# mohammed-amr/detectInBlur

Measured on AMD Instinct MI355X. Metric: blurred imgs/sec @800x1333 (--gpu_blur sparse correlation, fp16, batch 8), higher is better.
Workload: dtype f16; 1 GPU; configs[1]: --gpu_blur batch=8 3x800x1333 fp16, param_index=1 (expl 0.005), low_exposure fractions {1/18,1/10,1/5}, bit-exact accumulation; batch_per_gpu=8, parallelism=image-parallel x1

## Files before the change

### detectinblur_amd/csrc/dib_blur.hip

```cpp
#include "dib_compact_dev.h"
#include <mutex>
#include <stdlib.h>
#include <string.h>

extern "C" { __device__ __attribute__((used)) unsigned *dib_status_word = nullptr; }
#define DIB_STATUS_HANDOFF 1u
#define DIB_STATUS_GEOMETRY 2u
#define DIB_STATUS_WORDS 16
#ifdef DIB_STEP_POLLSTATS
extern "C" { __device__ __attribute__((used)) unsigned dib_poll_stats[4] = {0, 0, 0, 0}; }
#endif

namespace dib {

__device__ __forceinline__ void report_and_exit(unsigned code, unsigned detail) {
  typedef __attribute__((address_space(1))) unsigned gu32;
  gu32 *st = (gu32 *)(size_t)*(unsigned *volatile *)&dib_status_word;
  __hip_atomic_store(st + 1, detail, __ATOMIC_RELAXED, __HIP_MEMORY_SCOPE_SYSTEM);
  __hip_atomic_store(st, code, __ATOMIC_RELAXED, __HIP_MEMORY_SCOPE_SYSTEM);
  __builtin_amdgcn_endpgm();
}

typedef _Float16 h2 __attribute__((ext_vector_type(2)));
typedef unsigned uvec2 __attribute__((ext_vector_type(2)));
// ... 330 lines not shown

__device__ __forceinline__ bool band_entry(int T, int x, int t, int &local) {
  const int lo = (x * T) >> 3, hi = ((x + 1) * T) >> 3;
  local = lo + t;
  return t < hi - lo;
}
__device__ __forceinline__ void tile_of_local(const ImageDesc &d, int local, int &ch, int &tx, int &ty) {
  const int per_ch = d.tiles_x * d.tiles_y;
  ch = magic_div(local, d.inv_per_ch);
  local -= ch * per_ch;
  ty = magic_div(local, d.inv_tiles_x);
  tx = local - ty * d.tiles_x;
}
__device__ __forceinline__ bool tile_of_entry(const ImageDesc &d, int list, int entry, int &ch, int &tx, int &ty) {
  int local;
  if (!band_entry(d.C * d.tiles_x * d.tiles_y, list, entry, local)) return false;
  tile_of_local(d, local, ch, tx, ty);
  return true;
}
__device__ __forceinline__ void pin_desc(const ImageDesc &d) {
  asm volatile("" ::"s"(d.in), "s"(d.out), "s"(d.C), "s"(d.H), "s"(d.W), "s"(d.table), "s"(d.tiles_x), "s"(d.tiles_y),
               "s"(d.inv_per_ch), "s"(d.inv_tiles_x), "s"(d.tab));
}

constexpr int QTILE_W = 128;
constexpr int QPITCH = QUAD_PITCH * 8;
constexpr int QLDS_BYTES = LROWS * QPITCH;
static_assert(QPITCH == 448, "the asm below hard-codes the LDS row pitch");
static_assert(LROWS % NW == 0, "every wave fills the same number of window rows");
template <bool L> struct QGeom {
  static constexpr int PITCH_EL = L ? QUAD_PITCH_L : QUAD_PITCH;
  static constexpr int PITCH = PITCH_EL * 8;
  static constexpr int ROWS = TH + (L ? SEG_ROWS_L : SEG_ROWS);
  static constexpr int GQ = ROWS / NW;
  static constexpr int BYTES = ROWS * PITCH;
};
static_assert(QGeom<false>::PITCH == QPITCH && QGeom<false>::ROWS == LROWS && QGeom<false>::BYTES == QLDS_BYTES, "standard geometry");
static_assert(QGeom<true>::PITCH == 768 && QGeom<true>::ROWS % NW == 0 && QGeom<true>::BYTES == 39936, "the asm below hard-codes the large window's row pitch");

#define DIBQ_ADD(B, k) "v_pk_add_f16 %" #k ", %" #k ", v[" #B "+" #k "]\n\t"
#define DIBQ_MUL(B, k, W) "v_pk_mul_f16 v[" #B "+" #k "], " W ", v[" #B "+" #k "] op_sel:[1,0] op_sel_hi:[1,1]\n\t"
#define DIBQ_FMA(B, k, W) "v_pk_fma_f16 %" #k ", " W ", v[" #B "+" #k "], %" #k " op_sel:[1,0,0] op_sel_hi:[1,1,1]\n\t"
#define DIBQ_MADD(B, W) DIBQ_MUL(B, 0, W) DIBQ_MUL(B, 1, W) DIBQ_MUL(B, 2, W) DIBQ_MUL(B, 3, W) DIBQ_MUL(B, 4, W) DIBQ_MUL(B, 5, W) DIBQ_MUL(B, 6, W) DIBQ_MUL(B, 7, W) \
  DIBQ_ADD(B, 0) DIBQ_ADD(B, 1) DIBQ_ADD(B, 2) DIBQ_ADD(B, 3) DIBQ_ADD(B, 4) DIBQ_ADD(B, 5) DIBQ_ADD(B, 6) DIBQ_ADD(B, 7)
#define DIBQ_FMADD(B, W) DIBQ_FMA(B, 0, W) DIBQ_FMA(B, 1, W) DIBQ_FMA(B, 2, W) DIBQ_FMA(B, 3, W) DIBQ_FMA(B, 4, W) DIBQ_FMA(B, 5, W) DIBQ_FMA(B, 6, W) DIBQ_FMA(B, 7, W)
#define DIBQ_MADDH(B, W) DIBQ_MUL(B, 0, W) DIBQ_MUL(B, 2, W) DIBQ_MUL(B, 4, W) DIBQ_MUL(B, 6, W) DIBQ_ADD(B, 0) DIBQ_ADD(B, 2) DIBQ_ADD(B, 4) DIBQ_ADD(B, 6)
#define DIBQ_FMADDH(B, W) DIBQ_FMA(B, 0, W) DIBQ_FMA(B, 2, W) DIBQ_FMA(B, 4, W) DIBQ_FMA(B, 6, W)
#define DIBQ_READ(base, OFF, ADDR, P1, P2, P3)                                                                \
  "v_mad_u32_u16 v48, " OFF ", 1, " ADDR "\n\t"                                                               \
  "ds_read_b64 v[" #base ":" #base "+1], v48\n\tds_read_b64 v[" #base "+2:" #base "+3], v48 offset:" P1 "\n\t"  \
  "ds_read_b64 v[" #base "+4:" #base "+5], v48 offset:" P2 "\n\tds_read_b64 v[" #base "+6:" #base "+7], v48 offset:" P3 "\n\t"
#define DIBQ_READH(base, OFF, ADDR, P1, P2, P3)                                                               \
  "v_mad_u32_u16 v48, " OFF ", 1, " ADDR "\n\t"                                                               \
  "ds_read_b32 v[" #base "], v48\n\tds_read_b32 v[" #base "+2], v48 offset:" P1 "\n\t"                         \
  "ds_read_b32 v[" #base "+4], v48 offset:" P2 "\n\tds_read_b32 v[" #base "+6], v48 offset:" P3 "\n\t"
#define DIBQ_PITCH "448", "896", "1344"
#define DIBQ_PITCH_L "768", "1536", "2304"
#define DIBQ_LOAD(PAIR, LT, TOFF) "s_load_dwordx2 " PAIR ", " LT ", " TOFF "\n\ts_add_u32 " TOFF ", " TOFF ", 8\n\t"
#define DIBQ_NEXT(CNT, LABEL) "s_sub_u32 " CNT ", " CNT ", 1\n\ts_cbranch_scc1 " LABEL "\n\t"
#define DIBQ_LOOP6(PFX, TOFF, CNT, LT, ARITH, RD, ...) \
  DIBQ_LOAD("s[36:37]", LT, TOFF) DIBQ_LOAD("s[38:39]", LT, TOFF) "s_waitcnt vmcnt(0) lgkmcnt(0)\n\t" RD(32, "s36", __VA_ARGS__) \
  "L" PFX "_loop%=:\n\t" \
  "s_waitcnt lgkmcnt(0)\n\t" DIBQ_LOAD("s[40:41]", LT, TOFF) RD(40, "s37", __VA_ARGS__) ARITH(32, "s36") DIBQ_NEXT(CNT, "L" PFX "_done%=") \
  "s_waitcnt lgkmcnt(0)\n\t" RD(32, "s38", __VA_ARGS__) ARITH(40, "s37") DIBQ_NEXT(CNT, "L" PFX "_done%=") \
  "s_waitcnt lgkmcnt(0)\n\t" DIBQ_LOAD("s[36:37]", LT, TOFF) RD(40, "s39", __VA_ARGS__) ARITH(32, "s38") DIBQ_NEXT(CNT, "L" PFX "_done%=") \
  "s_waitcnt lgkmcnt(0)\n\t" RD(32, "s40", __VA_ARGS__) ARITH(40, "s39") DIBQ_NEXT(CNT, "L" PFX "_done%=") \
  "s_waitcnt lgkmcnt(0)\n\t" DIBQ_LOAD("s[38:39]", LT, TOFF) RD(40, "s41", __VA_ARGS__) ARITH(32, "s40") DIBQ_NEXT(CNT, "L" PFX "_done%=") \
  "s_waitcnt lgkmcnt(0)\n\t" RD(32, "s36", __VA_ARGS__) ARITH(40, "s41") \
  "s_sub_u32 " CNT ", " CNT ", 1\n\ts_cbranch_scc0 L" PFX "_loop%=\n\t" \
  "L" PFX "_done%=:\n\t" \
  "s_waitcnt lgkmcnt(0)"
#define DIBQ_CLOBBERS \
  "v32", "v33", "v34", "v35", "v36", "v37", "v38", "v39", "v40", "v41", "v42", "v43", "v44", "v45", "v46", "v47", "v48", \
  "s36", "s37", "s38", "s39", "s40", "s41", "scc", "memory"
template <bool FUSED, bool HALF, bool L = false>
__device__ __forceinline__ void tap_loop_quad(h2 (&acc)[8], unsigned long long ltaps, int t0, int n, unsigned lane_addr) {
#ifdef DIB_PORTABLE_TAPS
  return portable_taps<FUSED, HALF, 4, L ? 768u : 448u>(acc, ltaps, t0, n, lane_addr);
#endif
  unsigned toff = (unsigned)__builtin_amdgcn_readfirstlane(t0 * 4), cnt = (unsigned)__builtin_amdgcn_readfirstlane(n - 1);
  unsigned a[8];
#pragma unroll
  for (int i = 0; i < 8; ++i) a[i] = __builtin_bit_cast(unsigned, acc[i]);
#define DIB_RQ_ASM(ARITH, RD, ...) \
  asm volatile(DIBQ_LOOP6("dibq", "%8", "%9", "%10", ARITH, RD, "%11", __VA_ARGS__) \
      : "+v"(a[0]), "+v"(a[1]), "+v"(a[2]), "+v"(a[3]), "+v"(a[4]), "+v"(a[5]), "+v"(a[6]), "+v"(a[7]), "+s"(toff), "+s"(cnt) \
      : "s"(ltaps), "v"(lane_addr) \
      : DIBQ_CLOBBERS)
#define DIB_RQ_PICK(...) \
  if constexpr (FUSED && HALF) { DIB_RQ_ASM(DIBQ_FMADDH, DIBQ_READH, __VA_ARGS__); } \
  else if constexpr (FUSED) { DIB_RQ_ASM(DIBQ_FMADD, DIBQ_READ, __VA_ARGS__); } \
  else if constexpr (HALF) { DIB_RQ_ASM(DIBQ_MADDH, DIBQ_READH, __VA_ARGS__); } \
  else { DIB_RQ_ASM(DIBQ_MADD, DIBQ_READ, __VA_ARGS__); }
  if constexpr (L) { DIB_RQ_PICK(DIBQ_PITCH_L) } else { DIB_RQ_PICK(DIBQ_PITCH) }
#undef DIB_RQ_PICK
#undef DIB_RQ_ASM
#pragma unroll
  for (int i = 0; i < 8; ++i) acc[i] = __builtin_bit_cast(h2, a[i]);
}

#define DIBF_MIX(B, k, i, hs, W) "v_fma_mix_f32 %" #i ", " W ", v[" #B "+" #k "], %" #i " op_sel:[1," #hs ",0] op_sel_hi:[1,1,0]\n\t"
#define DIBF_ROWS(B, W) DIBF_MIX(B, 0, 0, 0, W) DIBF_MIX(B, 0, 1, 1, W) DIBF_MIX(B, 1, 2, 0, W) DIBF_MIX(B, 1, 3, 1, W) DIBF_MIX(B, 2, 4, 0, W) DIBF_MIX(B, 2, 5, 1, W) DIBF_MIX(B, 3, 6, 0, W) DIBF_MIX(B, 3, 7, 1, W) \
  DIBF_MIX(B, 4, 8, 0, W) DIBF_MIX(B, 4, 9, 1, W) DIBF_MIX(B, 5, 10, 0, W) DIBF_MIX(B, 5, 11, 1, W) DIBF_MIX(B, 6, 12, 0, W) DIBF_MIX(B, 6, 13, 1, W) DIBF_MIX(B, 7, 14, 0, W) DIBF_MIX(B, 7, 15, 1, W)
#define DIBF_ROWSH(B, W) DIBF_MIX(B, 0, 0, 0, W) DIBF_MIX(B, 0, 1, 1, W) DIBF_MIX(B, 2, 4, 0, W) DIBF_MIX(B, 2, 5, 1, W) DIBF_MIX(B, 4, 8, 0, W) DIBF_MIX(B, 4, 9, 1, W) DIBF_MIX(B, 6, 12, 0, W) DIBF_MIX(B, 6, 13, 1, W)
template <bool HALF, bool L>
__device__ __forceinline__ void tap_loop_quad_fp32(float (&acc)[16], unsigned long long ltaps, int t0, int n, unsigned lane_addr) {
#ifdef DIB_PORTABLE_TAPS
  {
    constexpr unsigned PITCH_B = L ? 768u : 448u;
    const unsigned *lt = reinterpret_cast<const unsigned *>(ltaps);
    for (int t = t0; t < t0 + n; ++t) {
      const unsigned word = lt[t];
      const float w = (float)half_of(word >> 16);
      const unsigned at = lane_addr + (word & 0xffffu);
#pragma unroll
      for (int i = 0; i < 4; ++i) {
        uvec2 e;
        if constexpr (HALF) { e.x = lds_b32(at + PITCH_B * i); e.y = 0; } else e = lds_b64(at + PITCH_B * i);
        acc[4 * i] = __builtin_fmaf(w, (float)half_of(e.x), acc[4 * i]);
        acc[4 * i + 1] = __builtin_fmaf(w, (float)half_of(e.x >> 16), acc[4 * i + 1]);
        if constexpr (!HALF) {
          acc[4 * i + 2] = __builtin_fmaf(w, (float)half_of(e.y), acc[4 * i + 2]);
          acc[4 * i + 3] = __builtin_fmaf(w, (float)half_of(e.y >> 16), acc[4 * i + 3]);
        }
      }
    }
    return;
  }
#endif
  unsigned toff = (unsigned)__builtin_amdgcn_readfirstlane(t0 * 4), cnt = (unsigned)__builtin_amdgcn_readfirstlane(n - 1);
#define DIB_RF_ASM(ARITH, RD, ...) \
  asm volatile(DIBQ_LOOP6("dibf", "%16", "%17", "%18", ARITH, RD, "%19", __VA_ARGS__) \
      : "+v"(acc[0]), "+v"(acc[1]), "+v"(acc[2]), "+v"(acc[3]), "+v"(acc[4]), "+v"(acc[5]), "+v"(acc[6]), "+v"(acc[7]), "+v"(acc[8]), \
        "+v"(acc[9]), "+v"(acc[10]), "+v"(acc[11]), "+v"(acc[12]), "+v"(acc[13]), "+v"(acc[14]), "+v"(acc[15]), "+s"(toff), "+s"(cnt) \
      : "s"(ltaps), "v"(lane_addr) \
      : DIBQ_CLOBBERS)
  if constexpr (L && HALF) { DIB_RF_ASM(DIBF_ROWSH, DIBQ_READH, DIBQ_PITCH_L); }
  else if constexpr (L) { DIB_RF_ASM(DIBF_ROWS, DIBQ_READ, DIBQ_PITCH_L); }
  else if constexpr (HALF) { DIB_RF_ASM(DIBF_ROWSH, DIBQ_READH, DIBQ_PITCH); }
  else { DIB_RF_ASM(DIBF_ROWS, DIBQ_READ, DIBQ_PITCH); }
#undef DIB_RF_ASM
}

#define VR_LO "op_sel:[0,0,0] op_sel_hi:[0,1,1]"
#define VR_HI "op_sel:[1,0,0] op_sel_hi:[1,1,1]"
#define VR_FMA(i, W, SEL, B, k) "v_pk_fma_f16 %" #i ", " W ", v[" #B "+" #k "], %" #i " " SEL "\n\t"
#define VR_TAP(B, j, W, SEL) VR_FMA(0, W, SEL, B, 2*j) VR_FMA(1, W, SEL, B, 2*j+1) VR_FMA(2, W, SEL, B, 2*j+2) VR_FMA(3, W, SEL, B, 2*j+3) \
  VR_FMA(4, W, SEL, B, 2*j+4) VR_FMA(5, W, SEL, B, 2*j+5) VR_FMA(6, W, SEL, B, 2*j+6) VR_FMA(7, W, SEL, B, 2*j+7)
#define VR_TAPH(B, j, W, SEL) VR_FMA(0, W, SEL, B, 2*j) VR_FMA(2, W, SEL, B, 2*j+2) VR_FMA(4, W, SEL, B, 2*j+4) VR_FMA(6, W, SEL, B, 2*j+6)
#define VR_RD(B, k, off) "ds_read_b64 v[" #B "+2*" #k ":" #B "+2*" #k "+1], v60 offset:" #off "\n\t"
#define VR_RDH(B, k, off) "ds_read_b32 v[" #B "+2*" #k "], v60 offset:" #off "\n\t"
#define VR_READS4(RD, B, OFF) "v_mad_u32_u16 v60, " OFF ", 1, %10\n\t" RD(B, 0, 0) RD(B, 1, 448) RD(B, 2, 896) RD(B, 3, 1344) RD(B, 4, 1792) RD(B, 5, 2240) RD(B, 6, 2688)
#define VR_READS3(RD, B, OFF) "v_mad_u32_u16 v60, " OFF ", 1, %10\n\t" RD(B, 0, 0) RD(B, 1, 448) RD(B, 2, 896) RD(B, 3, 1344) RD(B, 4, 1792) RD(B, 5, 2240)
#define VR_READS2(RD, B, OFF) "v_mad_u32_u16 v60, " OFF ", 1, %10\n\t" RD(B, 0, 0) RD(B, 1, 448) RD(B, 2, 896) RD(B, 3, 1344) RD(B, 4, 1792)
#define VR_READS1(RD, B, OFF) "v_mad_u32_u16 v60, " OFF ", 1, %10\n\t" RD(B, 0, 0) RD(B, 1, 448) RD(B, 2, 896) RD(B, 3, 1344)
#define VR_ARITH4(TAP, B, W01, W23) TAP(B, 3, W23, VR_HI) TAP(B, 2, W23, VR_LO) TAP(B, 1, W01, VR_HI) TAP(B, 0, W01, VR_LO)
#define VR_ARITH3(TAP, B, W01, W23) TAP(B, 2, W23, VR_LO) TAP(B, 1, W01, VR_HI) TAP(B, 0, W01, VR_LO)
#define VR_ARITH2(TAP, B, W01, W23) TAP(B, 1, W01, VR_HI) TAP(B, 0, W01, VR_LO)
#define VR_ARITH1(TAP, B, W01, W23) TAP(B, 0, W01, VR_LO)
#define VR_STEP(N, NM1, RD, TAP, BC, BN, C0, C1, C2, OTHER, P, Q)                                            \
  "Lvr_c" #N P "%=:\n\t"                                                                                    \
  "s_waitcnt lgkmcnt(0)\n\t"                                                                                \
  "s_load_dwordx4 " OTHER ", %9, %8\n\ts_add_u32 %8, %8, 16\n\t"                                            \
  VR_READS##N(RD, BN, C0)                                                                                   \
  "s_bfe_u32 s46, " C0 ", 0x30010\n\t"                                                                      \
  VR_ARITH##N(TAP, BC, C1, C2)                                                                              \
  "s_cmp_eq_u32 s46, " NM1 "\n\ts_cbranch_scc1 Lvr_c" #N Q "%=\n\t"                                         \
  "s_branch Lvr_d" Q "%=\n\t"
#define VR_BODY(N, NM1, RD, TAP)                                                                             \
  VR_STEP(N, NM1, RD, TAP, 32, 46, "s36", "s37", "s38", "s[40:43]", "x", "y")                               \
  VR_STEP(N, NM1, RD, TAP, 46, 32, "s40", "s41", "s42", "s[36:39]", "y", "x")
#define VR_DISPATCH(P)                                                                                       \
  "Lvr_d" P "%=:\n\t"                                                                                       \
  "s_cmp_eq_u32 s46, 4\n\ts_cbranch_scc1 Lvr_done%=\n\t"                                                    \
  "s_cmp_eq_u32 s46, 3\n\ts_cbranch_scc1 Lvr_c4" P "%=\n\t"                                                 \
  "s_cmp_eq_u32 s46, 2\n\ts_cbranch_scc1 Lvr_c3" P "%=\n\t"                                                 \
  "s_cmp_eq_u32 s46, 1\n\ts_cbranch_scc1 Lvr_c2" P "%=\n\t"                                                 \
  "s_branch Lvr_c1" P "%=\n\t"
template <bool HALF>
__device__ __forceinline__ void tap_loop_quad_vrun(h2 (&acc)[8], unsigned long long vgroups, int g0, unsigned lane_addr) {
#ifdef DIB_PORTABLE_TAPS
  {
    const uint4 *rec = reinterpret_cast<const uint4 *>(vgroups) + g0;
    uint4 r = rec[0];
    unsigned off = r.w & 0xffffu, code = (r.w >> 16) & 7u;
    for (int g = 0;; ++g) {
      const int n = (int)code + 1;
      uvec2 row[7];
#pragma unroll
      for (int k = 0; k < 7; ++k) {
        row[k] = uvec2{0u, 0u};
        if (k < n + 3) { if constexpr (HALF) row[k].x = lds_b32(lane_addr + off + 448u * k); else row[k] = lds_b64(lane_addr + off + 448u * k); }
      }
#pragma unroll
      for (int j = 3; j >= 0; --j) {
        if (j >= n) continue;
        const _Float16 w = half_of((j < 2 ? r.y : r.z) >> (16 * (j & 1)));
#pragma unroll
        for (int i = 0; i < 4; ++i) {
          acc[2 * i] = tap_pk<true>(acc[2 * i], row[j + i].x, w);
          if constexpr (!HALF) acc[2 * i + 1] = tap_pk<true>(acc[2 * i + 1], row[j + i].y, w);
        }
      }
      off = r.x & 0xffffu; code = (r.x >> 16) & 7u;
      if (code == 4u) break;
      r = rec[g + 1];
    }
    return;
  }
#endif
  unsigned toff = (unsigned)__builtin_amdgcn_readfirstlane(g0 * 16);
  unsigned a[8];
#pragma unroll
  for (int i = 0; i < 8; ++i) a[i] = __builtin_bit_cast(unsigned, acc[i]);
#define DIB_VR_ASM(RD, TAP) \
  asm volatile( \
       \
      "s_load_dwordx4 s[36:39], %9, %8\n\ts_add_u32 %8, %8, 16\n\t" \
      "s_waitcnt vmcnt(0) lgkmcnt(0)\n\t" \
      "s_bfe_u32 s46, s39, 0x30010\n\t" \
      VR_READS4(RD, 32, "s39") \
      "s_branch Lvr_dx%=\n\t" \
      VR_BODY(4, "3", RD, TAP) VR_BODY(3, "2", RD, TAP) VR_BODY(2, "1", RD, TAP) VR_BODY(1, "0", RD, TAP) \
      VR_DISPATCH("x") VR_DISPATCH("y") \
      "Lvr_done%=:\n\t" \
      "s_waitcnt lgkmcnt(0)" \
      : "+v"(a[0]), "+v"(a[1]), "+v"(a[2]), "+v"(a[3]), "+v"(a[4]), "+v"(a[5]), "+v"(a[6]), "+v"(a[7]), "+s"(toff) \
      : "s"(vgroups), "v"(lane_addr) \
      : "v32", "v33", "v34", "v35", "v36", "v37", "v38", "v39", "v40", "v41", "v42", "v43", "v44", "v45", "v46", "v47", "v48", "v49", "v50", \
        "v51", "v52", "v53", "v54", "v55", "v56", "v57", "v58", "v59", "v60", "s36", "s37", "s38", "s39", "s40", "s41", "s42", "s43", "s46", \
        "scc", "memory")
  if constexpr (HALF) { DIB_VR_ASM(VR_RDH, VR_TAPH); }
  else { DIB_VR_ASM(VR_RD, VR_TAP); }
#undef DIB_VR_ASM
#pragma unroll
  for (int i = 0; i < 8; ++i) acc[i] = __builtin_bit_cast(h2, a[i]);
}

struct NoWait { __device__ void operator()() const {} };
struct NormArgs {
  float mean[MAX_BATCH][4], std[MAX_BATCH][4];
  int Hp, Wp;
  int nhwc;
};
__device__ __forceinline__ unsigned lds_addr(unsigned *shared) { return (unsigned)(size_t)(__attribute__((address_space(3))) char *)shared; }
template <int ACC, bool L = false, bool STEP = false, typename Wait = NoWait, bool NORM = false>
__device__ __forceinline__ void blur_quad_tile_f16(const ImageDesc &d, const int *__restrict__ tab, int K, int ch, int tx, int ty,
                                                   const unsigned lds0, const int wave, const int early = 0, const int nsegs0 = 0,
                                                   const uint4 seg0 = uint4{0, 0, 0, 0}, const Wait wait_tables = Wait(),
                                                   const NormArgs *na = nullptr, const int img = 0) {
#pragma clang fp contract(off)
  constexpr int GQ = QGeom<L>::GQ;
  constexpr int QPITCH = QGeom<L>::PITCH, QUAD_PITCH = QGeom<L>::PITCH_EL, LROWS = QGeom<L>::ROWS;
  const int H = d.H, W = d.W, w2 = W * 2;
  const int mode = pad_mode_for(K, H, W);
  const int pb = K / 2 - 1, pa = K / 2;
  const uint4 *segs = reinterpret_cast<const uint4 *>(tab + table_segs_off(K));
  int nsegs;
  int use_vruns = 0;
  uint4 seg;
  if (STEP && early) {
    nsegs = nsegs0 | 1 << 30;
    seg = seg0;
  } else {
    unsigned __int128 r, hd;
    asm volatile("s_load_dwordx4 %0, %2, 0x10\n\ts_load_dwordx4 %1, %3, 0x0\n\ts_waitcnt lgkmcnt(0)"
                 : "=&s"(hd), "=&s"(r) : "s"((unsigned long long)tab), "s"((unsigned long long)segs));
    seg = make_uint4((unsigned)r, (unsigned)(r >> 32), (unsigned)(r >> 64), (unsigned)(r >> 96));
    nsegs = (int)(unsigned)(hd >> 96);
    if constexpr (!STEP) {
      const unsigned kw = (unsigned)(hd >> 32) >> 16;
      if ((kw & 1u) != (L ? 1u : 0u)) report_and_exit(DIB_STATUS_GEOMETRY, (unsigned)(hd >> 32));
      if constexpr (ACC == DIB_ACC_FAST16) use_vruns = (int)(kw >> 1) & 1;
    }
  }
  static_assert(HDR_NSEGS == 7 && HDR_K == 5 && HDR_WORDS == 8, "header words 4..7 in the asm above");
  const unsigned long long ltaps = uniform64((unsigned long long)(tab + table_ltaps_q_off(K)));
  const int x0c = tx * QTILE_W, y0c = ty * TH, pxy = ty << 16 | tx;
  auto x0f = [&]() -> int { if constexpr (STEP) { int p = pxy; asm volatile("" : "+s"(p)); return (p & 0xffff) * QTILE_W; } else return x0c; };
  auto y0f = [&]() -> int { if constexpr (STEP) { int p = pxy; asm volatile("" : "+s"(p)); return (int)((unsigned)p >> 16) * TH; } else return y0c; };
  const __amdgpu_buffer_rsrc_t in_rsrc = plane_rsrc(d.in, ch, H, W);
  h2 acc[8];
  float acc32[16];
#pragma unroll
  for (int i = 0; i < 8; ++i) acc[i] = h2{0, 0};
#pragma unroll
  for (int i = 0; i < 16; ++i) acc32[i] = 0.f;
  const int qb = wave * GQ;
  auto fresh_lane = [&]() { int l; asm volatile("v_mbcnt_lo_u32_b32 %0, -1, 0\n\tv_mbcnt_hi_u32_b32 %0, -1, %0" : "=v"(l)); return l; };

#ifdef DIB_TIMELINE
#define DIB_TL_STAMP(WHEN, SLOT) \
  if (!L && !STEP && WHEN && wave == 0 && fresh_lane() == 0) \
    *(__attribute__((address_space(3))) unsigned long long *)(size_t)(lds0 + QGeom<false>::BYTES + SLOT) = __builtin_amdgcn_s_memrealtime()
#else
#define DIB_TL_STAMP(WHEN, SLOT)
#endif
  DIB_TL_STAMP(true, 32);
  for (int sg = 0; sg < (STEP ? (nsegs & 0xffffff) : nsegs); ++sg) {
    if (sg > 0) seg = segs[sg];
    const Window w = window_of(seg);
    const int lane = fresh_lane();
    const int x0 = x0f(), y0 = y0f();
    constexpr int NK = L ? 6 : 4;
    constexpr int PARTS = (ACC == DIB_ACC_FP32 && !L) ? 2 : 1, GP = (GQ + PARTS - 1) / PARTS;
    short v[GP][NK];
    unsigned coff[NK];
    int soff[GQ];
    unsigned zmask = 0;
    const int c_first = x0 + pb - w.cmax, r_first = y0 + pb - w.rl;
    const bool zero_mode = mode == PAD_ZERO;
    if (!zero_mode && c_first >= 0 && c_first + 63 + 32 * (NK - 1) <= W - 1) {
      const unsigned c0 = 2u * (unsigned)(c_first + lane);
#pragma unroll
      for (int k = 0; k < NK; ++k) coff[k] = c0 + 64u * k;
    } else {
#pragma unroll
      for (int k = 0; k < NK; ++k) {
        bool z;
        coff[k] = 2u * (unsigned)map_coord_sel(c_first + lane + 32 * k, W, pa, pb, mode, z);
        zmask |= z ? 1u << k : 0u;
      }
    }
    if (!zero_mode && r_first >= 0 && r_first + LROWS - 1 <= H - 1) {
      const int s0 = (r_first + qb) * w2;
#pragma unroll
      for (int g = 0; g < GQ; ++g) soff[g] = s0 + g * w2;
    } else {
      const int nrows = TH + (w.rl - w.rf);
#pragma unroll
      for (int g = 0; g < GQ; ++g) {
        bool zr;
        const int sr = map_coord_sel(r_first + min(qb + g, nrows - 1), H, pa, pb, mode, zr);
        zmask |= zr ? 1u << (8 + g) : 0u;
        soff[g] = sr * w2;
      }
    }
    const bool masked = __builtin_amdgcn_ballot_w64(zmask != 0) != 0;
#pragma unroll
    for (int part = 0; part < PARTS; ++part) {
#pragma unroll
      for (int g = 0; g < GP; ++g) {
        if (part * GP + g >= GQ) continue;
        const int so = __builtin_amdgcn_readfirstlane(soff[part * GP + g]);
#pragma unroll
        for (int k = 0; k < NK; ++k) v[g][k] = __builtin_amdgcn_raw_buffer_load_b16(in_rsrc, coff[k], so, 0);
      }
      DIB_TL_STAMP(sg == 0 && part == 0, 40);
      if (part == 0 && sg > 0) __syncthreads();
      const int wl = fresh_lane();
      const unsigned wp = lds0 + (unsigned)((qb + part * GP) * QPITCH + wl * 8);
      if constexpr (L) {
#pragma unroll
        for (int g = 0; g < GP; ++g) {
          if (part * GP + g >= GQ) continue;
          unsigned u[NK];
#pragma unroll
          for (int k = 0; k < NK; ++k)
            u[k] = (masked && (((zmask >> k) & 1u) || ((zmask >> (8 + part * GP + g)) & 1u))) ? 0u : (unsigned)(unsigned short)v[g][k];
          uvec2 e;
          e.x = u[0] | (u[1] << 16);
          e.y = u[2] | (u[3] << 16);
          *(lds_u2 *)(size_t)(wp + (unsigned)(g * QPITCH)) = e;
          if (wl < 32) {
            uvec2 f;
            f.x = u[2] | (u[3] << 16);
            f.y = u[4] | (u[5] << 16);
            *(lds_u2 *)(size_t)(wp + (unsigned)(g * QPITCH + 512)) = f;
          }
        }
      } else if (wl < QUAD_PITCH) {
        if (!masked) {
#pragma unroll
          for (int g = 0; g < GP; ++g) {
            if (part * GP + g >= GQ) continue;
            uvec2 e;
            typedef short s2v __attribute__((ext_vector_type(2)));
            e.x = __builtin_bit_cast(unsigned, s2v{v[g][0], v[g][1]});
            e.y = __builtin_bit_cast(unsigned, s2v{v[g][2], v[g][3]});
            *(lds_u2 *)(size_t)(wp + (unsigned)(g * QPITCH)) = e;
          }
        } else {
#pragma unroll
          for (int g = 0; g < GP; ++g) {
            if (part * GP + g >= GQ) continue;
            unsigned u[4];
#pragma unroll
            for (int k = 0; k < 4; ++k)
              u[k] = (((zmask >> k) & 1u) || ((zmask >> (8 + part * GP + g)) & 1u)) ? 0u : (unsigned)(unsigned short)v[g][k];
            uvec2 e;
            e.x = u[0] | (u[1] << 16);
            e.y = u[2] | (u[3] << 16);
            *(lds_u2 *)(size_t)(wp + (unsigned)(g * QPITCH)) = e;
          }
        }
      }
    }
    __syncthreads();
    DIB_TL_STAMP(sg == 0, 16);
    if constexpr (STEP) { if (sg == 0 && (nsegs >> 30)) wait_tables(); }
    const int tl = fresh_lane();
    const unsigned lane_addr = lds0 + (unsigned)((wave * 8 + (tl >> 5) * 4) * QPITCH + (tl & 31) * 8);
    if constexpr (ACC == DIB_ACC_FP32) {
      if (W - x0f() <= 64) tap_loop_quad_fp32<true, L>(acc32, ltaps, w.t0, w.n, lane_addr);
      else tap_loop_quad_fp32<false, L>(acc32, ltaps, w.t0, w.n, lane_addr);
    } else if constexpr (ACC == DIB_ACC_FAST16) {
      const unsigned long long vg = uniform64((unsigned long long)(tab + table_vgroups_off(K)));
      if (!use_vruns) {
        if (W - x0f() <= 64) tap_loop_quad<true, true, L>(acc, ltaps, w.t0, w.n, lane_addr);
        else tap_loop_quad<true, false, L>(acc, ltaps, w.t0, w.n, lane_addr);
      } else if (W - x0f() <= 64) tap_loop_quad_vrun<true>(acc, vg, w.t0, lane_addr);
      else tap_loop_quad_vrun<false>(acc, vg, w.t0, lane_addr);
    } else {
      if (W - x0f() <= 64) tap_loop_quad<ACC == DIB_ACC_FMA16, true, L>(acc, ltaps, w.t0, w.n, lane_addr);
      else tap_loop_quad<ACC == DIB_ACC_FMA16, false, L>(acc, ltaps, w.t0, w.n, lane_addr);
    }
  }
  if constexpr (ACC == DIB_ACC_FP32) {
#pragma unroll
    for (int i = 0; i < 8; ++i) acc[i] = h2{(_Float16)acc32[2 * i], (_Float16)acc32[2 * i + 1]};
  }
  DIB_TL_STAMP(true, 24);
#undef DIB_TL_STAMP
  if constexpr (NORM) {
    const int Hp = na->Hp, Wp = na->Wp, nhwc = na->nhwc;
    const float m = na->mean[img][ch], sd = na->std[img][ch];
    const unsigned long long a = uniform64((unsigned long long)d.out + (nhwc ? (unsigned long long)ch * 4ull : (unsigned long long)ch * Hp * Wp * 4ull));
    const __amdgpu_buffer_rsrc_t out_rsrc = __builtin_amdgcn_make_buffer_rsrc((void *)a, 0, Hp * Wp * 4 * (nhwc ? 3 : 1) - (nhwc ? ch * 4 : 0), 0x00020000);
    const int x0 = x0f(), y0 = y0f();
    const int sl = fresh_lane();
    const int yl = y0 + wave * 8 + (sl >> 5) * 4, xl = x0 + (sl & 31);
    const unsigned px = nhwc ? 12u : 4u;
    const unsigned base = (unsigned)(yl * Wp + xl) * px, oob = 0x7ffffff0u;
    const bool inside = x0 + QTILE_W <= W && y0 + TH <= H;
#pragma unroll
    for (int i = 0; i < 4; ++i) {
      const unsigned ro = base + (unsigned)(i * Wp) * px;
      const float v[4] = {(float)acc[2 * i].x, (float)acc[2 * i].y, (float)acc[2 * i + 1].x, (float)acc[2 * i + 1].y};
#pragma unroll
      for (int q = 0; q < 4; ++q) {
        const int col = xl + 32 * q, row = yl + i;
        const bool in_img = inside || (row < H && col < W);
        const float f = in_img ? (v[q] - m) / sd : 0.f;
        __builtin_amdgcn_raw_buffer_store_b32(__builtin_bit_cast(int, f), out_rsrc, (in_img || (row < Hp && col < Wp)) ? ro + 32u * q * px : oob, 0, 0);
      }
    }
  } else {
    int chs = ch;
    if constexpr (STEP) asm volatile("" : "+s"(chs));
    const __amdgpu_buffer_rsrc_t out_rsrc = plane_rsrc(d.out, chs, H, W);
    const int x0 = x0f(), y0 = y0f();
    const int sl = fresh_lane();
    const int yl = y0 + wave * 8 + (sl >> 5) * 4, xl = x0 + (sl & 31);
    const unsigned base = (unsigned)(yl * w2 + xl * 2), oob = 0x7ffffff0u;
    if (x0 + QTILE_W <= W && y0 + TH <= H) {
      typedef int i4v __attribute__((ext_vector_type(4)));
      const unsigned long long pa2 = uniform64((unsigned long long)d.out + (unsigned long long)chs * H * W * 2ull);
      const i4v rs = {(int)(unsigned)pa2, (int)(unsigned)(pa2 >> 32) & 0xffff, H * W * 2, 0x00020000};
      int so = 0;
#pragma unroll
      for (int i = 0; i < 4; ++i) {
        asm volatile("buffer_store_short %0, %2, %3, %4 offen\n\t"
                     "buffer_store_short_d16_hi %0, %2, %3, %4 offen offset:64\n\t"
                     "buffer_store_short %1, %2, %3, %4 offen offset:128\n\t"
                     "buffer_store_short_d16_hi %1, %2, %3, %4 offen offset:192"
                     :: "v"(acc[2 * i]), "v"(acc[2 * i + 1]), "v"(base), "s"(rs), "s"(so) : "memory");
        so += w2;
      }
      return;
    }
#pragma unroll
    for (int i = 0; i < 4; ++i) {
      const bool row_ok = yl + i < H;
      const unsigned a0 = __builtin_bit_cast(unsigned, acc[2 * i]), a1 = __builtin_bit_cast(unsigned, acc[2 * i + 1]);
      const unsigned ro = base + (unsigned)(i * w2);
      __builtin_amdgcn_raw_buffer_store_b16((short)(a0 & 0xffffu), out_rsrc, row_ok && xl < W ? ro : oob, 0, 0);
      __builtin_amdgcn_raw_buffer_store_b16((short)(a0 >> 16), out_rsrc, row_ok && xl + 32 < W ? ro + 64u : oob, 0, 0);
      __builtin_amdgcn_raw_buffer_store_b16((short)(a1 & 0xffffu), out_rsrc, row_ok && xl + 64 < W ? ro + 128u : oob, 0, 0);
      __builtin_amdgcn_raw_buffer_store_b16((short)(a1 >> 16), out_rsrc, row_ok && xl + 96 < W ? ro + 192u : oob, 0, 0);
    }
  }
}

#ifdef DIB_TIMELINE
__device__ unsigned long long *g_timeline;
#define DIB_TL_SLOT (*(unsigned long long *volatile *)&g_timeline)
constexpr int TL_WORD = QLDS_BYTES / 4;
#endif

template <int ACC, int KC, bool FLAT = false>
__global__ __launch_bounds__(256, 8) void blur_quad_f16_kernel(BlurBatch batch, FlatBands fb) {
  constexpr int K = KC;
  extern __shared__ unsigned nlds[];
  int img_i = blockIdx.y, entry = blockIdx.x >> 3;
  if constexpr (FLAT) {
    typedef int i16v __attribute__((ext_vector_type(16)));
    const i16v bb = *reinterpret_cast<const i16v *>(fb.begin[blockIdx.x & 7]);
    const int len = bb[15];
    if (entry >= len) return;
    {
      const int row = entry >> 5, full = len >> 5;
      if (row < full && row < 32 && ((fb.rev_mask >> row) & 1u)) entry ^= 31;
    }
    int start = bb[0];
    img_i = 0;
#pragma unroll
    for (int k = 1; k < FLAT_MAX; ++k) {
      const bool ge = entry >= bb[k];
      img_i += ge ? 1 : 0;
      start = ge ? bb[k] : start;
    }
    entry -= start;
  }
#ifdef DIB_TIMELINE
  if (threadIdx.x == 0) {
    *(unsigned long long *)(nlds + TL_WORD) = __builtin_amdgcn_s_memrealtime();
    nlds[TL_WORD + 2] = FLAT ? blockIdx.x : blockIdx.y * 1024 + blockIdx.x;
    nlds[TL_WORD + 3] = img_i;
  }
#endif
  const ImageDesc d = batch.img[img_i];
  pin_desc(d);
  int ch, tx, ty;
  if (!tile_of_entry(d, blockIdx.x & 7, entry, ch, tx, ty)) return;
  blur_quad_tile_f16<ACC>(d, d.tab, K, ch, tx, ty, lds_addr(nlds), __builtin_amdgcn_readfirstlane((int)threadIdx.x >> 6));
#ifdef DIB_TIMELINE
  if (threadIdx.x == 0) {
    unsigned long long *tl = DIB_TL_SLOT;
    if (tl) {
      asm volatile("s_waitcnt vmcnt(0)" ::: "memory");
      unsigned long long *o = tl + 8 * (size_t)*(volatile unsigned *)(nlds + TL_WORD + 2);
      o[0] = *(volatile unsigned long long *)(nlds + TL_WORD);
      o[1] = __builtin_amdgcn_s_memrealtime();
      o[2] = __builtin_amdgcn_s_getreg((31 << 11) | 4);
      o[3] = (unsigned long long)__builtin_amdgcn_s_getreg((31 << 11) | 20) | (unsigned long long)*(volatile unsigned *)(nlds + TL_WORD + 3) << 32;
      o[4] = *(volatile unsigned long long *)(nlds + TL_WORD + 4); o[5] = *(volatile unsigned long long *)(nlds + TL_WORD + 6);
      o[6] = *(volatile unsigned long long *)(nlds + TL_WORD + 8); o[7] = *(volatile unsigned long long *)(nlds + TL_WORD + 10);
    }
  }
#endif
}

constexpr unsigned STEP_EARLY = 4096;
constexpr int STEP_LDS_EXTRA = 16;
#ifdef DIB_STEP_STAMPS
__device__ unsigned long long *g_step_stamps;
#endif
struct StepWait {
  unsigned lds_words;
  __device__ __forceinline__ void operator()() const {
    static_assert(STEP_REPLICA_WORDS * 4 == 128, "the shift below");
#ifdef DIB_PORTABLE_TAPS
    {
      const uvec2 sp = lds_b64(lds_words), tb = lds_b64(lds_words + 8);
      const unsigned xcc = __builtin_amdgcn_s_getreg((2 << 11) | 20);
      const unsigned *ctr = reinterpret_cast<const unsigned *>((((unsigned long long)(unsigned)__builtin_amdgcn_readfirstlane((int)sp.y) << 32) |
                                                                 (unsigned)__builtin_amdgcn_readfirstlane((int)sp.x)) + 128ull * xcc);
      const unsigned target = (unsigned)__builtin_amdgcn_readfirstlane((int)tb.x), budget = (unsigned)__builtin_amdgcn_readfirstlane((int)tb.y);
      for (unsigned spins = 0;; ++spins) {
        if ((int)(__hip_atomic_load(ctr, __ATOMIC_RELAXED, __HIP_MEMORY_SCOPE_AGENT) - target) >= 0) return;
        if (spins >= budget) report_and_exit(DIB_STATUS_HANDOFF, target);
        __builtin_amdgcn_s_sleep(2);
      }
    }
#endif
    asm volatile(
        "v_mov_b32 v48, %0\n\t"
        "ds_read_b64 v[46:47], v48\n\t"
        "ds_read_b64 v[44:45], v48 offset:8\n\t"
        "s_getreg_b32 s39, hwreg(20, 0, 3)\n\t"
        "s_lshl_b32 s39, s39, 7\n\t"
        "s_waitcnt lgkmcnt(0)\n\t"
        "v_readfirstlane_b32 s36, v46\n\t"
        "v_readfirstlane_b32 s37, v47\n\t"
        "v_readfirstlane_b32 s38, v44\n\t"
        "s_add_u32 s36, s36, s39\n\t"
        "s_addc_u32 s37, s37, 0\n\t"
        "v_readfirstlane_b32 s39, v45\n\t"
        "s_load_dword s40, s[36:37], 0x0\n\t"
        "s_mov_b32 s41, 0\n\t"
        "s_waitcnt lgkmcnt(0)\n\t"
        "s_sub_u32 s40, s40, s38\n\t"
        "s_cmp_lt_i32 s40, 0\n\t"
        "s_cbranch_scc0 Ldibw_done%=\n\t"
        "v_mov_b32 v48, 0\n\t"
        "Ldibw_poll%=:\n\t"
        "global_load_dword v48, v48, s[36:37] sc1\n\t"
        "s_waitcnt vmcnt(0)\n\t"
        "v_readfirstlane_b32 s40, v48\n\t"
        "v_mov_b32 v48, 0\n\t"
        "s_sub_u32 s40, s40, s38\n\t"
        "s_cmp_lt_i32 s40, 0\n\t"
        "s_cbranch_scc0 Ldibw_done%=\n\t"
        "s_sleep 2\n\t"
        "s_add_u32 s41, s41, 1\n\t"
        "s_cmp_lt_u32 s41, s39\n\t"
        "s_cbranch_scc1 Ldibw_poll%=\n\t"
        "s_getpc_b64 s[36:37]\n\t"
        "s_add_u32 s36, s36, dib_status_word@rel32@lo+4\n\t"
        "s_addc_u32 s37, s37, dib_status_word@rel32@hi+12\n\t"
        "s_load_dwordx2 s[36:37], s[36:37], 0x0\n\t"
        "v_mov_b32 v47, s38\n\t"
        "v_mov_b32 v46, 1\n\t"
        "s_waitcnt lgkmcnt(0)\n\t"
        "global_store_dword v48, v47, s[36:37] offset:4 sc0 sc1\n\t"
        "global_store_dword v48, v46, s[36:37] sc0 sc1\n\t"
        "s_waitcnt vmcnt(0)\n\t"
        "s_endpgm\n\t"
        "Ldibw_done%=:\n\t"
#ifdef DIB_STEP_POLLSTATS
        "s_cmp_lt_u32 s41, 33\n\t"
        "s_cbranch_scc1 Ldibw_nostat%=\n\t"
        "s_getpc_b64 s[36:37]\n\t"
        "s_add_u32 s36, s36, dib_poll_stats@rel32@lo+4\n\t"
        "s_addc_u32 s37, s37, dib_poll_stats@rel32@hi+12\n\t"
        "v_mov_b32 v48, 0\n\t"
        "global_load_dword v47, v48, s[36:37] offset:4 sc1\n\t"
        "s_waitcnt vmcnt(0)\n\t"
        "v_readfirstlane_b32 s40, v47\n\t"
        "s_cmp_le_u32 s41, s40\n\t"
        "s_cbranch_scc1 Ldibw_nostat%=\n\t"
        "v_mov_b32 v47, s41\n\t"
        "global_atomic_umax v48, v47, s[36:37] offset:4\n\t"
        "Ldibw_nostat%=:\n\t"
#endif
        :: "s"(lds_words)
        : "s36", "s37", "s38", "s39", "s40", "s41", "v44", "v45", "v46", "v47", "v48", "scc", "memory");
  }
};
static_assert(DIB_STATUS_HANDOFF == 1u, "the v_mov_b32 v46, 1 above");

template <int ACC>
__global__ __launch_bounds__(256, 8) void blur_step_f16_kernel(BlurBatch batch, StepSync sy, PsfPtrs psfs) {
  constexpr int K = 128;
  extern __shared__ unsigned nlds[];
  const ImageDesc d = batch.img[blockIdx.y];
  asm volatile("" ::"s"(d.in), "s"(d.out), "s"(d.C), "s"(d.H), "s"(d.W), "s"(d.table), "s"(d.tiles_x), "s"(d.tiles_y),
               "s"(d.inv_per_ch), "s"(d.inv_tiles_x), "s"(d.tab), "s"(sy.sync), "s"(sy.target), "s"(sy.ncx), "s"(sy.row), "s"(sy.rec));
  const int wave = __builtin_amdgcn_readfirstlane((int)threadIdx.x >> 6);
  if (blockIdx.x < (unsigned)sy.ncx) {
    if (blockIdx.y == 0 && blockIdx.x < (unsigned)sy.n_psf && !(sy.flags & COMPACT_DEBUG_NOSIGNAL)) {
      unsigned *rec = sy.rec + (size_t)blockIdx.x * (STEP_REPLICAS * STEP_REC_WORDS);
#ifdef DIB_STEP_STAMPS
      unsigned long long *dbg = *(unsigned long long *volatile *)&g_step_stamps;
      if (dbg) dbg += 8 * blockIdx.x;
      compact_psf_f16_wg256<true, true>(psfs.p[blockIdx.x], sy.flags, sy.tables + (size_t)blockIdx.x * table_words(K), (lds_u32 *)nlds, wave, rec, sy.target, dbg);
#else
      compact_psf_f16_wg256<true, true>(psfs.p[blockIdx.x], sy.flags, sy.tables + (size_t)blockIdx.x * table_words(K), (lds_u32 *)nlds, wave, rec, sy.target);
#endif
      asm volatile("s_waitcnt vmcnt(0)" ::: "memory");
      __syncthreads();
      const int t = wave * 64 + (int)__builtin_amdgcn_mbcnt_hi(~0u, __builtin_amdgcn_mbcnt_lo(~0u, 0u));
#ifdef DIB_STEP_STAMPS
      if (dbg && t == 0) dbg[6] = __builtin_amdgcn_s_memrealtime();
#endif
      if (t < STEP_REPLICAS)
        __hip_atomic_fetch_add(sy.sync + t * STEP_REPLICA_WORDS, 1u, __ATOMIC_RELAXED, __HIP_MEMORY_SCOPE_AGENT);
#ifdef DIB_STEP_STAMPS
      asm volatile("s_waitcnt vmcnt(0)" ::: "memory");
      if (dbg && t == 0) dbg[7] = __builtin_amdgcn_s_memrealtime();
#endif
    }
    return;
  }
  const unsigned bx = blockIdx.x - (unsigned)sy.ncx;
  const int per_ch = d.tiles_x * d.tiles_y;
  int local;
  if (!band_entry(d.C * per_ch, bx & 7, bx >> 3, local)) __builtin_amdgcn_endpgm();
#ifdef DIB_STEP_STAMPS
  unsigned long long *bdbg = *(unsigned long long *volatile *)&g_step_stamps;
  if (bdbg && blockIdx.y == 0 && wave == 0) { bdbg += 8 * MAX_BATCH + 4 * bx; bdbg[0] = __builtin_amdgcn_s_memrealtime(); } else bdbg = nullptr;
#endif
  int early = 1;
  if (blockIdx.y * (unsigned)sy.row + blockIdx.x >= STEP_EARLY) {
    unsigned c;
    asm volatile("s_load_dword %0, %1, 0x0\n\ts_waitcnt lgkmcnt(0)" : "=s"(c) : "s"(sy.sync + (blockIdx.x & 7) * STEP_REPLICA_WORDS) : "memory");
    early = (int)((c - sy.target) >> 31);
  }
  asm volatile("" : "+s"(early));
  int nsegs0 = 0;
  uint4 seg0 = make_uint4(0, 0, 0, 0);
  if (early) {
    const unsigned long long *pr = reinterpret_cast<const unsigned long long *>(sy.rec + ((size_t)d.table * STEP_REPLICAS + (blockIdx.x & (STEP_REPLICAS - 1))) * STEP_REC_WORDS);
#ifdef DIB_STEP_POLLSTATS
    unsigned pspins = 0;
#endif
    for (unsigned spins = 0;; ++spins) {
#ifdef DIB_STEP_POLLSTATS
      pspins = spins;
#endif
      const unsigned long long ra = __hip_atomic_load(pr, __ATOMIC_RELAXED, __HIP_MEMORY_SCOPE_AGENT);
      const unsigned long long rb = __hip_atomic_load(pr + 1, __ATOMIC_RELAXED, __HIP_MEMORY_SCOPE_AGENT);
      const unsigned ta = __builtin_amdgcn_readfirstlane((unsigned)(ra >> 32)), tb = __builtin_amdgcn_readfirstlane((unsigned)(rb >> 32));
      if (ta == sy.target && tb == sy.target) {
        const unsigned a = __builtin_amdgcn_readfirstlane((unsigned)ra), b2 = __builtin_amdgcn_readfirstlane((unsigned)rb);
        nsegs0 = (int)(a >> 16);
// ... 597 lines not shown
```

Measured before the change: 185,300 images/s.

## Remap non-L quad fill to half-wave row pairs and skip rows beyond window

For the non-L tile fill path, each half-wave now loads one row using 32 lanes over five column strips. Lanes 0-23 write a second shifted quad element, which replaces the old scheme of 64 lanes over four strips with lanes idle above QUAD_PITCH. Row iterations beyond the window's actual row count (trim_rows) are skipped, so short kernels load and store fewer halo rows. Row offsets are folded into the column offsets when the tile is fully inside the image. This adds complexity and per-lane row mapping in the boundary path.

```diff
diff --git a/detectinblur_amd/csrc/dib_blur.hip b/detectinblur_amd/csrc/dib_blur.hip
--- a/detectinblur_amd/csrc/dib_blur.hip
+++ b/detectinblur_amd/csrc/dib_blur.hip
@@ -656,96 +656,170 @@
     const Window w = window_of(seg);
     const int lane = fresh_lane();
     const int x0 = x0f(), y0 = y0f();
-    constexpr int NK = L ? 6 : 4;
-    constexpr int PARTS = (ACC == DIB_ACC_FP32 && !L) ? 2 : 1, GP = (GQ + PARTS - 1) / PARTS;
-    short v[GP][NK];
-    unsigned coff[NK];
-    int soff[GQ];
-    unsigned zmask = 0;
     const int c_first = x0 + pb - w.cmax, r_first = y0 + pb - w.rl;
     const bool zero_mode = mode == PAD_ZERO;
-    if (!zero_mode && c_first >= 0 && c_first + 63 + 32 * (NK - 1) <= W - 1) {
-      const unsigned c0 = 2u * (unsigned)(c_first + lane);
-#pragma unroll
-      for (int k = 0; k < NK; ++k) coff[k] = c0 + 64u * k;
-    } else {
-#pragma unroll
-      for (int k = 0; k < NK; ++k) {
-        bool z;
-        coff[k] = 2u * (unsigned)map_coord_sel(c_first + lane + 32 * k, W, pa, pb, mode, z);
-        zmask |= z ? 1u << k : 0u;
+    unsigned zmask = 0;
+    if constexpr (L) {
+      constexpr int NK = 6;
+      short v[GQ][NK];
+      unsigned coff[NK];
+      int soff[GQ];
+      if (!zero_mode && c_first >= 0 && c_first + 63 + 32 * (NK - 1) <= W - 1) {
+        const unsigned c0 = 2u * (unsigned)(c_first + lane);
+#pragma unroll
+        for (int k = 0; k < NK; ++k) coff[k] = c0 + 64u * k;
+      } else {
+#pragma unroll
+        for (int k = 0; k < NK; ++k) {
+          bool z;
+          coff[k] = 2u * (unsigned)map_coord_sel(c_first + lane + 32 * k, W, pa, pb, mode, z);
+          zmask |= z ? 1u << k : 0u;
+        }
       }
-    }
-    if (!zero_mode && r_first >= 0 && r_first + LROWS - 1 <= H - 1) {
-      const int s0 = (r_first + qb) * w2;
-#pragma unroll
-      for (int g = 0; g < GQ; ++g) soff[g] = s0 + g * w2;
-    } else {
-      const int nrows = TH + (w.rl - w.rf);
+      if (!zero_mode && r_first >= 0 && r_first + LROWS - 1 <= H - 1) {
+        const int s0 = (r_first + qb) * w2;
+#pragma unroll
+        for (int g = 0; g < GQ; ++g) soff[g] = s0 + g * w2;
+      } else {
+        const int nrows = TH + (w.rl - w.rf);
+#pragma unroll
+        for (int g = 0; g < GQ; ++g) {
+          bool zr;
+          const int sr = map_coord_sel(r_first + min(qb + g, nrows - 1), H, pa, pb, mode, zr);
+          zmask |= zr ? 1u << (8 + g) : 0u;
+          soff[g] = sr * w2;
+        }
+      }
+      const bool masked = __builtin_amdgcn_ballot_w64(zmask != 0) != 0;
 #pragma unroll
       for (int g = 0; g < GQ; ++g) {
-        bool zr;
-        const int sr = map_coord_sel(r_first + min(qb + g, nrows - 1), H, pa, pb, mode, zr);
-        zmask |= zr ? 1u << (8 + g) : 0u;
-        soff[g] = sr * w2;
-      }
-    }
-    const bool masked = __builtin_amdgcn_ballot_w64(zmask != 0) != 0;
-#pragma unroll
-    for (int part = 0; part < PARTS; ++part) {
-#pragma unroll
-      for (int g = 0; g < GP; ++g) {
-        if (part * GP + g >= GQ) continue;
-        const int so = __builtin_amdgcn_readfirstlane(soff[part * GP + g]);
+        const int so = __builtin_amdgcn_readfirstlane(soff[g]);
 #pragma unroll
         for (int k = 0; k < NK; ++k) v[g][k] = __builtin_amdgcn_raw_buffer_load_b16(in_rsrc, coff[k], so, 0);
       }
-      DIB_TL_STAMP(sg == 0 && part == 0, 40);
-      if (part == 0 && sg > 0) __syncthreads();
+      if (sg > 0) __syncthreads();
       const int wl = fresh_lane();
-      const unsigned wp = lds0 + (unsigned)((qb + part * GP) * QPITCH + wl * 8);
-      if constexpr (L) {
-#pragma unroll
-        for (int g = 0; g < GP; ++g) {
-          if (part * GP + g >= GQ) continue;
-          unsigned u[NK];
-#pragma unroll
-          for (int k = 0; k < NK; ++k)
-            u[k] = (masked && (((zmask >> k) & 1u) || ((zmask >> (8 + part * GP + g)) & 1u))) ? 0u : (unsigned)(unsigned short)v[g][k];
-          uvec2 e;
-          e.x = u[0] | (u[1] << 16);
-          e.y = u[2] | (u[3] << 16);
-          *(lds_u2 *)(size_t)(wp + (unsigned)(g * QPITCH)) = e;
-          if (wl < 32) {
-            uvec2 f;
-            f.x = u[2] | (u[3] << 16);
-            f.y = u[4] | (u[5] << 16);
-            *(lds_u2 *)(size_t)(wp + (unsigned)(g * QPITCH + 512)) = f;
+      const unsigned wp = lds0 + (unsigned)(qb * QPITCH + wl * 8);
+#pragma unroll
+      for (int g = 0; g < GQ; ++g) {
+        unsigned u[NK];
+#pragma unroll
+        for (int k = 0; k < NK; ++k)
+          u[k] = (masked && (((zmask >> k) & 1u) || ((zmask >> (8 + g)) & 1u))) ? 0u : (unsigned)(unsigned short)v[g][k];
+        uvec2 e;
+        e.x = u[0] | (u[1] << 16);
+        e.y = u[2] | (u[3] << 16);
+        *(lds_u2 *)(size_t)(wp + (unsigned)(g * QPITCH)) = e;
+        if (wl < 32) {
+          uvec2 f;
+          f.x = u[2] | (u[3] << 16);
+          f.y = u[4] | (u[5] << 16);
+          *(lds_u2 *)(size_t)(wp + (unsigned)(g * QPITCH + 512)) = f;
+        }
+      }
+    } else {
+      constexpr int NI = (LROWS + 2 * NW - 1) / (2 * NW), PARTS = ACC == DIB_ACC_FP32 ? 2 : 1, IP = NI / PARTS;
+      static_assert(NI == 6 && NI % PARTS == 0 && QUAD_PITCH - 32 == 24, "six iterations in one or two parts; lanes 0-23 of a half-wave write a second element");
+      short v[IP][5];
+      unsigned coff[5];
+      const int nrows = TH + (w.rl - w.rf);
+#ifdef DIB_FILL_NOTRIM
+      int trim_rows = LROWS;
+      asm volatile("" : "+s"(trim_rows));
+#else
+      const int trim_rows = nrows;
+#endif
+      auto skipped = [&](int i) { return i >= TH / 8 && (8 * i >= trim_rows || 8 * i + 2 * wave >= LROWS); };
+      if (!zero_mode && c_first >= 0 && c_first + 31 + 32 * 4 <= W - 1) {
+        const unsigned c0 = 2u * (unsigned)(c_first + (lane & 31));
+#pragma unroll
+        for (int k = 0; k < 5; ++k) coff[k] = c0 + 64u * k;
+      } else {
+#pragma unroll
+        for (int k = 0; k < 5; ++k) {
+          bool z;
+          coff[k] = 2u * (unsigned)map_coord_sel(c_first + (lane & 31) + 32 * k, W, pa, pb, mode, z);
+          zmask |= z ? 1u << k : 0u;
+        }
+      }
+      const int rows_touched = min((trim_rows + 7) & ~7, LROWS);
+      const bool rows_inside = !zero_mode && r_first >= 0 && r_first + rows_touched - 1 <= H - 1;
+      if (rows_inside) {
+        const unsigned r0 = (unsigned)((r_first + 2 * wave + (lane >> 5)) * w2);
+#pragma unroll
+        for (int k = 0; k < 5; ++k) coff[k] += r0;
+      }
+#pragma unroll
+      for (int part = 0; part < PARTS; ++part) {
+        if (rows_inside) {
+#pragma unroll
+          for (int j = 0; j < IP; ++j) {
+            const int i = part * IP + j;
+            if (skipped(i)) continue;
+            const int so = 8 * i * w2;
+#pragma unroll
+            for (int k = 0; k < 5; ++k) v[j][k] = __builtin_amdgcn_raw_buffer_load_b16(in_rsrc, coff[k], so, 0);
+          }
+        } else {
+#pragma unroll
+          for (int j = 0; j < IP; ++j) {
+            const int i = part * IP + j;
+            if (skipped(i)) continue;
+            bool zr;
+            const int sr = map_coord_sel(r_first + min(8 * i + 2 * wave + (lane >> 5), nrows - 1), H, pa, pb, mode, zr);
+            zmask |= zr ? 1u << (8 + i) : 0u;
+            const unsigned ro = (unsigned)(sr * w2);
+#pragma unroll
+            for (int k = 0; k < 5; ++k) v[j][k] = __builtin_amdgcn_raw_buffer_load_b16(in_rsrc, coff[k] + ro, 0, 0);
           }
         }
-      } else if (wl < QUAD_PITCH) {
+        const bool masked = __builtin_amdgcn_ballot_w64(zmask != 0) != 0;
+        DIB_TL_STAMP(sg == 0 && part == 0, 40);
+        if (part == 0 && sg > 0) __syncthreads();
+        const int wl = fresh_lane();
+        const unsigned wp = lds0 + (unsigned)((2 * wave + (wl >> 5)) * QPITCH + (wl & 31) * 8);
+        const bool second = (wl & 31) < QUAD_PITCH - 32;
+        typedef short s2v __attribute__((ext_vector_type(2)));
         if (!masked) {
 #pragma unroll
-          for (int g = 0; g < GP; ++g) {
-            if (part * GP + g >= GQ) continue;
+          for (int j = 0; j < IP; ++j) {
+            const int i = part * IP + j;
+            if (skipped(i)) continue;
             uvec2 e;
-            typedef short s2v __attribute__((ext_vector_type(2)));
-            e.x = __builtin_bit_cast(unsigned, s2v{v[g][0], v[g][1]});
-            e.y = __builtin_bit_cast(unsigned, s2v{v[g][2], v[g][3]});
-            *(lds_u2 *)(size_t)(wp + (unsigned)(g * QPITCH)) = e;
+            e.x = __builtin_bit_cast(unsigned, s2v{v[j][0], v[j][1]});
+            e.y = __builtin_bit_cast(unsigned, s2v{v[j][2], v[j][3]});
+            *(lds_u2 *)(size_t)(wp + (unsigned)(8 * i * QPITCH)) = e;
+          }
+          if (second) {
+#pragma unroll
+            for (int j = 0; j < IP; ++j) {
+              const int i = part * IP + j;
+              if (skipped(i)) continue;
+              uvec2 f;
+              f.x = __builtin_bit_cast(unsigned, s2v{v[j][1], v[j][2]});
+              f.y = __builtin_bit_cast(unsigned, s2v{v[j][3], v[j][4]});
+              *(lds_u2 *)(size_t)(wp + (unsigned)(8 * i * QPITCH + 256)) = f;
+            }
           }
         } else {
 #pragma unroll
-          for (int g = 0; g < GP; ++g) {
-            if (part * GP + g >= GQ) continue;
-            unsigned u[4];
-#pragma unroll
-            for (int k = 0; k < 4; ++k)
-              u[k] = (((zmask >> k) & 1u) || ((zmask >> (8 + part * GP + g)) & 1u)) ? 0u : (unsigned)(unsigned short)v[g][k];
+          for (int j = 0; j < IP; ++j) {
+            const int i = part * IP + j;
+            if (skipped(i)) continue;
+            unsigned u[5];
+#pragma unroll
+            for (int k = 0; k < 5; ++k)
+              u[k] = (((zmask >> k) & 1u) || ((zmask >> (8 + i)) & 1u)) ? 0u : (unsigned)(unsigned short)v[j][k];
             uvec2 e;
             e.x = u[0] | (u[1] << 16);
             e.y = u[2] | (u[3] << 16);
-            *(lds_u2 *)(size_t)(wp + (unsigned)(g * QPITCH)) = e;
+            *(lds_u2 *)(size_t)(wp + (unsigned)(8 * i * QPITCH)) = e;
+            if (second) {
+              uvec2 f;
+              f.x = u[1] | (u[2] << 16);
+              f.y = u[3] | (u[4] << 16);
+              *(lds_u2 *)(size_t)(wp + (unsigned)(8 * i * QPITCH + 256)) = f;
+            }
           }
         }
       }
```

Measured after the change: 186,500 images/s (median of 6 runs). About the same (+0.7%).
